# VatsalSy/gerris-fft-particles

Hardware: AMD Instinct MI355X
Metric: Mcell-steps/s (projection+advection), 3D 256^3 uniform (higher is better)
Workload: dtype f64; 1 GPU; 3-D periodic Taylor-Green, 256^3 per GPU, default projection/advection parameters (SURVEY 8d config C); relax_mode=exact, parallelism=1 box, rccl_world_size=0

## Files before the change

### gerris-fft-particles_amd/csrc/gfship_internal.hpp

```cpp
#pragma once

#include <hip/hip_runtime.h>
#include <cstdio>
#include <cstdarg>
#include <cstring>
#include <vector>
#include <deque>
#include <string>
#include <type_traits>
#include "gfship.h"
#include "switches.hpp"
#include "cell_update.hpp"

namespace gfship {

struct Layout {
  int n = 0;
  int px = 0;
  int xo = 1;
  int rows = 0;
  int dim = 3;
  long sy = 0;
  long sz = 0;
  size_t total = 0;
  __host__ __device__ inline long idx (int i, int j, int k) const {
    return xo + i + sy*j + sz*k;
  }
};

struct Field {
  bool used = false;
  int component = -1;
  double * lev[GFSHIP_MAXLEVEL + 1] = {};
  int bc[6] = {0, 0, 0, 0, 0, 0};
  double * bcval[6] = {};
// ... 69 lines not shown
  void * comm = nullptr;
  int overlap = 0;
  int lat_rank = -1, lat_n = 0, lat_b[3] = { 1, 1, 1 };
  gfship_gather_fn gather = nullptr; void * gather_ctx = nullptr;
  double * lat_res = nullptr, * lat_xch = nullptr;
  unsigned * lat_bar = nullptr;
  size_t lat_res_doubles = 0, lat_xch_doubles = 0;
  double * gfv_send[6] = {}, * gfv_recv[6] = {};
  double src[3] = { 0., 0., 0. };
  unsigned long long n_lattice_cycles = 0, n_fused_mpi = 0;
  unsigned long long kc[GFSHIP_KC_COUNT] = {};
  bool lattice_attr_set = false;
  void * mpi_plan[GFSHIP_MAXLEVEL + 1] = {};
  gfship_field dp_cache = -1;
  int skew_resident = -1;
  int patch_resident = 0;
  bool no_fused_godunov = false;
  bool no_fused_loop = false;
  bool force_hyperplane = false;
  bool unit_weights = false;
  bool weighted = false;
  unsigned long weights_stamp = 0;
  gfship_field wf[6] = {-1, -1, -1, -1, -1, -1};
  gfship::SkewPlan skew[GFSHIP_MAXLEVEL + 1];
  double diff_w[GFSHIP_MAXLEVEL + 1] = {};
  double * cfl_partial = nullptr;
  size_t cfl_nblocks = 0, cfl_used = 0;
  bool cfl_dirty = false;
  bool coarse_attr_set = false;
  gfship_field res_cache = -1;
  bool diff_ready = false;
  int diff_kind = 1;
  int patch_call = -1;
};

namespace gfship {

void set_error (const char * fmt, ...);
int  hip_fail (hipError_t e, const char * what, const char * file, int line);

inline int before_write (gfship_domain * dom)
{
  return dom->before_write ? dom->before_write (dom->before_write_ctx) : GFSHIP_OK;
}

#define GFSHIP_HIP(call) do { hipError_t e_ = (call); \
    if (e_ != hipSuccess) return gfship::hip_fail (e_, #call, __FILE__, __LINE__); } while (0)

inline hipError_t stream_wait_spin (hipStream_t st)
{
  hipError_t e;
  while ((e = hipStreamQuery (st)) == hipErrorNotReady)
    ;
  return e;
}

template <class F> inline void with_bools (F && f) { f (); }
template <class F, class... B> inline void with_bools (F && f, bool b0, B... rest)
{
  if (b0) with_bools ([&] (auto... r) { f (std::true_type {}, r...); }, rest...);
  else    with_bools ([&] (auto... r) { f (std::false_type {}, r...); }, rest...);
}

template <class F, class... B> inline void with_kind (F && f, int kind, B... bools)
{
  auto k = [&] (auto K) { with_bools ([&] (auto... r) { f (K, r...); }, bools...); };
// ... 52 lines not shown
			    int (* after_shell) (void *), void * ctx);
void mpi_order_free (gfship_domain * dom);
int launch_relax_loop_small (gfship_domain * dom, unsigned dimension, int level, double omega,
			     Field * dp, Field * ubc, const double * rhs, const double * dia,
			     unsigned nrelax, bool * done, const RelaxOp * op = nullptr);
int coarse_cycle_top (gfship_domain * dom, int minlevel);
int lattice_cycle_top (gfship_domain * dom, int minlevel, Field * dia);
int lattice_check_error (gfship_domain * dom);
int launch_lattice_cycle (gfship_domain * dom, unsigned dimension, double omega, int lmin, int ltop,
			  const unsigned * nrelax, Field * dp, Field * ubc, Field * res);
int launch_coarse_cycle (gfship_domain * dom, unsigned dimension, double omega, int lmin, int ltop,
			 const unsigned * nrelax, Field * dp, Field * ubc, Field * res, Field * dia);
int launch_relax_redblack (gfship_domain * dom, unsigned dimension, int level, double omega,
			   double * u, const double * rhs, const double * dia);
int launch_residual (gfship_domain * dom, int level, const double * u, const double * rhs,
		     const double * dia, double * res);
int launch_residual_weighted (gfship_domain * dom, int level, const double * u, const double * rhs,
			      const double * dia, double * res);
int launch_poisson_weights (gfship_domain * dom, double * const alpha[3]);
int launch_diffusion_weights (gfship_domain * dom, double * const D[3], double cdt);
int alloc_weights (gfship_domain * dom);
RelaxOp weighted_op (gfship_domain * dom, int level);
int launch_restrict (gfship_domain * dom, unsigned dimension, int level_coarse, double * v_coarse,
		     const double * v_fine);
int launch_prolongate (gfship_domain * dom, int level_coarse, const double * v_coarse,
		       double * v_fine);
int launch_correct (gfship_domain * dom, int level, double * u, const double * dp);
int launch_fill (gfship_domain * dom, int level, double * a, double value);
int launch_residual_norm (gfship_domain * dom, int level, const double * u, const double * rhs,
			  const double * dia, double * res, double scale, double weight,
			  double * out , bool dia_zero = false,
			  bool * store = nullptr );
int launch_norm_async (gfship_domain * dom, int level, const double * a, double scale, double weight);

int poisson_solve (gfship_domain * dom, gfship_multilevel_params * par, gfship_field lhs, gfship_field rhs,
		   gfship_field res, gfship_field dia, double dt, bool res_unread);
int launch_norm (gfship_domain * dom, int level, const double * a, double scale, double weight,
		 double out[5] );

int launch_face_interp_un (gfship_domain * dom, double * const u[3], double * const un[3]);
int launch_divergence (gfship_domain * dom, double * const un[3], double * div, double dt);
int launch_correct_un (gfship_domain * dom, const double * p, double * const un[3], double dt);
int launch_centered_gradient (gfship_domain * dom, const double * p, double * const g[3]);
int launch_correct_centered (gfship_domain * dom, double * const u[3], double * const g[3], double dt);
int launch_correct_centered_coarse (gfship_domain * dom, double * const u[3], double * const g[3],
				    double dt, double * const uc[3]);
int launch_coarse_init_from (gfship_domain * dom, Field * const * v, int nf, int top);
int launch_coarse_init_levels (gfship_domain * dom, Field * const * v, int nf, int top, int bottom);
int launch_advected_face_values (gfship_domain * dom, const double * v, double * const u[3],
				 double * const un[3], double dt, int use_centered, int gradient,
				 double * const fv[6], int cmask, double visc = 0., double gsrc = 0.,
				 const double * msrc = nullptr );
int launch_variable_mac_source (gfship_domain * dom, const double * v, double * const D[3],
				const double * alpha, double * out);
int launch_mac_source_fields (gfship_domain * dom, int c, const double * F, bool add_out, double * out);
int launch_centered_source_fields (gfship_domain * dom, double * v, const double * F, double gsrc, double dt);
int launch_face_bc (gfship_domain * dom, Field * v, double * const fv[6], int cmask);
int launch_predict_un (gfship_domain * dom, int cc, const double * uc, double * const fv[6],
		       double * unc);
int launch_flux_update (gfship_domain * dom, bool velocity, double * v, double * const un[3],
			double * const fv[6], const double * gm, const double * gc, double dt,
			double gsrc = 0.);
int launch_cfl (gfship_domain * dom, double * const u[3], double * const un[3],
		const double visc[3], double * cfl2,
		double * const msrc[3] = nullptr );
int launch_coarse_init (gfship_domain * dom, Field * const * v, int nf);
// ... 27 lines not shown
int  launch_relax_loop_skew (gfship_domain * dom, int level, Field * dp, Field * ubc,
			     const double * rhs, const double * dia, bool dia_zero,
			     unsigned nrelax, bool bc, double * correct_into = nullptr,
			     const double * prolong_from = nullptr, const RelaxOp * op = nullptr);
void skew_free (gfship_domain * dom);
bool skew_loop_supported (gfship_domain * dom, int level, unsigned nrelax, bool bc);
struct LoopGhosts;
int  skew_loop_run (gfship_domain * dom, int level, SkewPlan * S, double * u_nat, bool has_dia,
		    unsigned nrelax, float * ms = nullptr, const Field * ubc = nullptr,
		    const RelaxOp * op = nullptr, LoopGhosts * ghosts = nullptr);
int  skew_time_loop (gfship_domain * dom, int level, Field * u, const double * rhs,
		     const double * dia, bool dia_zero, unsigned nrelax, int reps,
		     double * ms_per_loop, int * fused, double * ms_inclusive = nullptr);
int  skew_check_error (gfship_domain * dom);
int  skew_arm_ahead (gfship_domain * dom, int level, unsigned nrelax);
int  patch_resident_per_cu (const gfship_domain * dom);
bool prolongation_fused (gfship_domain * dom, unsigned dimension, int level, unsigned nrelax);
bool prolongation_fusable (gfship_domain * dom, unsigned dimension, int level, unsigned nrelax);
bool line_prolongation_fused (gfship_domain * dom, unsigned dimension, int level, unsigned nrelax);
bool line_prolongation_fusable (gfship_domain * dom, unsigned dimension, int level, unsigned nrelax);
inline bool patch_level (const gfship_domain * dom, int level)
{
  const bool per_cell_weights = dom->patch_call < 0 ? dom->weighted : dom->patch_call == 0;
  return dom->sw.patch () && !per_cell_weights && dom->lay[level].n >= dom->sw.patch_min_n;
}
int  patch_pack (gfship_domain * dom, int level, SkewPlan * S, const double * u, const double * rhs,
		 const double * dia, const double * coarse = nullptr);
int  patch_unpack (gfship_domain * dom, int level, SkewPlan * S, double * u, double * add_into,
		   const LoopGhosts * ghosts = nullptr);
int  patch_restrict_pack (gfship_domain * dom, int level, SkewPlan * S, const double * res,
			  double * res_coarse, SkewPlan * Sc, unsigned dimension);
int  launch_restrict_pack (gfship_domain * dom, unsigned dimension, int level, Field * res,
			   bool coarse_fused);
void skew_dump_stats (gfship_domain * dom, int level);
int  skew_time_sweeps (gfship_domain * dom, int level, Field * u, const double * rhs,
		       const double * dia, bool dia_zero, int reps, double * ms_per_sweep);

}
```

### gerris-fft-particles_amd/csrc/poisson.hip

```cpp
#include "gfship_internal.hpp"
#include <cmath>
#include <cfloat>
#include <cstdlib>

using namespace gfship;

#define GFSHIP_CHECK_DIMENSION(dom, d) \
  GFSHIP_CHECK ((d) == (unsigned) (dom)->dim, GFSHIP_EUNSUPPORTED, \
		"dimension %u on a %d-D domain: only the dimension of the domain is implemented", (d), (dom)->dim)

namespace gfship {

static bool weighted_pipelinable (gfship_domain * dom, unsigned dimension, int level)
{
  return dom->relax_mode == GFSHIP_RELAX_EXACT && dimension == 3 && dom->dim == 3 &&
    skew_supported (dom, level) && !dom->force_hyperplane;
}

static bool weighted_pipelined (gfship_domain * dom, unsigned dimension, int level)
{
  return dom->sw.weighted_pipelined && weighted_pipelinable (dom, dimension, level);
}

static int relax_level (gfship_domain * dom, unsigned dimension, int level, double omega,
// ... 262 lines not shown

int gfship_norm_variable (gfship_domain * dom, gfship_field v, gfship_norm * out)
{
  Field * V = get_field (dom, v);
  if (!V || !out) return GFSHIP_EINVAL;
  const Layout & L = dom->lay[dom->depth];
  double size = 1./L.n;
  double vol = dom->dim == 3 ? size*size*size : size*size;
  double s[5];
  int r = launch_norm (dom, dom->depth, V->lev[dom->depth], 1., vol, s);
  if (r) return r;
  gfship_norm n;
  double wv = vol*(double) ncells (L);
  if (dom->has_external) {
    double sums[4] = { s[0], s[1], s[2], wv }, mx[1] = { s[3] };
    if ((r = call_reduce_norm (dom, sums, 4, mx))) return r;
    s[0] = sums[0]; s[1] = sums[1]; s[2] = sums[2]; wv = sums[3]; s[3] = mx[0];
  }
  n.bias = s[0]; n.first = s[1]; n.second = s[2]; n.infty = s[3];
  n.w = wv;
  if (n.w > 0.) {
    n.bias /= n.w;
    n.first /= n.w;
    n.second = sqrt (n.second/n.w);
  }
  else
    n.infty = 0.;
  *out = n;
  return GFSHIP_OK;
}

}

static int poisson_cycle (gfship_domain * dom, gfship_multilevel_params * p,
			  gfship_field u, gfship_field rhs, gfship_field dia, gfship_field res,
			  double dt, gfship_norm * norm, bool * store_res = nullptr)
{
  GFSHIP_CHECK (dom && p, GFSHIP_EINVAL, "null argument");
  GFSHIP_CHECK (p->dimension == 2 || p->dimension == 3, GFSHIP_EINVAL, "dimension must be 2 or 3");
  GFSHIP_CHECK_DIMENSION (dom, p->dimension);
  GFSHIP_CHECK (p->nrelax > 0 && p->erelax > 0, GFSHIP_EINVAL, "nrelax and erelax must be non zero");
  GFSHIP_CHECK (dom->unit_weights, GFSHIP_EINVAL, "call gfship_poisson_coefficients first");
  if (dom->dp_cache < 0)
    dom->dp_cache = gfship_field_alloc (dom, -1);
  gfship_field dpf = dom->dp_cache;
  if (dpf < 0) return dpf;
  Field * U = get_field (dom, u), * R = get_field (dom, rhs), * D = get_field (dom, dia),
    * S = get_field (dom, res), * DP = get_field (dom, dpf);
  int r = GFSHIP_OK;
  bool corrected = false;
  if (!U || !R || !D || !S) return GFSHIP_EINVAL;
  const int L = dom->depth;
  unsigned minlevel = p->minlevel;
  if (minlevel > (unsigned) L) minlevel = L;
  p->depth = L;

#define TRY(x) do { if ((r = (x)) != GFSHIP_OK) goto done; } while (0)
  for (int l = 0; l <= L; l++)
    S->zero[l] = U->zero[l] = false;
  {
    unsigned nrl[GFSHIP_MAXLEVEL + 1];
    {
      unsigned nr = p->nrelax;
      for (int l = L; l >= 0; l--) {
	nrl[l] = nr;
	if (l > (int) minlevel) nr *= p->erelax;
      }
    }
    for (int l = 0; l <= L; l++)
      DP->zero[l] = false;
    const int ctop = dom->weighted ? -1 : coarse_cycle_top (dom, (int) minlevel);
    const int ltop = ctop >= 0 ? -1 : lattice_cycle_top (dom, (int) minlevel, D);
    for (int l = L - 1; l >= (ctop >= 0 ? ctop + 1 : ltop >= 0 ? ltop : 0); l--) {
      if (dom->relax_mode == GFSHIP_RELAX_EXACT && p->dimension == 3 && !dom->weighted &&
	  !dom->force_hyperplane && skew_supported (dom, l + 1))
	TRY (skew_arm_ahead (dom, l + 1, nrl[l + 1]));
      const bool rp = !dom->skew[l + 1].rs_ready && prolongation_fused (dom, p->dimension, l + 1, nrl[l + 1]);
      if (rp) dom->kc[dom->sw.fused_restriction ? GFSHIP_KC_RESTRICTION_FUSED : GFSHIP_KC_RESTRICTION_DECLINED]++;
      if (dom->sw.fused_restriction && rp)
	TRY (launch_restrict_pack (dom, p->dimension, l + 1, S,
				   l > (int) minlevel && prolongation_fused (dom, p->dimension, l, nrl[l])));
      else
	TRY (launch_restrict (dom, p->dimension, l, S->lev[l], S->lev[l + 1]));
    }
    unsigned first = minlevel;
    if (ltop >= 0) {
      TRY (launch_lattice_cycle (dom, p->dimension, p->omega, (int) minlevel, ltop, nrl, DP, U, S));
      first = ltop + 1;
    }
    else if (ctop >= 0) {
      TRY (launch_coarse_cycle (dom, p->dimension, p->omega, (int) minlevel, ctop, nrl, DP, U, S, D));
      first = ctop + 1;
    }
    else {
      TRY (launch_fill (dom, minlevel, DP->lev[minlevel], 0.));
      TRY (relax_loop (dom, DP, U, p->dimension, minlevel, p->omega, S, D, nrl[minlevel]));
      first = minlevel + 1;
      dom->kc[GFSHIP_KC_COARSE_END_BY_LEVEL]++;
    }
    for (unsigned l = first; l <= p->depth; l++) {
      const bool fp = prolongation_fused (dom, p->dimension, (int) l, nrl[l]) ||
	line_prolongation_fused (dom, p->dimension, (int) l, nrl[l]);
      if (fp) dom->kc[GFSHIP_KC_PROLONGATION_FUSED]++;
      else if (prolongation_fusable (dom, p->dimension, (int) l, nrl[l]) ||
	       line_prolongation_fusable (dom, p->dimension, (int) l, nrl[l]))
	dom->kc[GFSHIP_KC_PROLONGATION_DECLINED]++;
      if (!fp)
	TRY (launch_prolongate (dom, l - 1, DP->lev[l - 1], DP->lev[l]));
      TRY (relax_loop (dom, DP, U, p->dimension, l, p->omega, S, D, nrl[l],
		       (int) l == L ? U->lev[L] : nullptr, &corrected, fp ? DP->lev[l - 1] : nullptr));
    }
  }
  if (!corrected)
    TRY (launch_correct (dom, L, U->lev[L], DP->lev[L]));
  if (!(corrected && all_sides_periodic (dom)))
    TRY (launch_bc (dom, U, U, L, 0));
  if (norm)
    TRY (residual_and_norm (dom, dt, U, R, D, S, norm, store_res));
  else if (dom->weighted)
    TRY (launch_residual_weighted (dom, L, U->lev[L], R->lev[L], D->lev[L], S->lev[L]));
  else
    TRY (launch_residual (dom, L, U->lev[L], R->lev[L], D->lev[L], S->lev[L]));
#undef TRY
 done:
  for (int l = 0; l <= L; l++)
    dom->skew[l].rs_ready = false;
  return r;
}

extern "C" {

int gfship_poisson_cycle (gfship_domain * dom, gfship_multilevel_params * p,
			  gfship_field u, gfship_field rhs, gfship_field dia, gfship_field res)
{
  GFSHIP_CHECK (dom != nullptr, GFSHIP_EINVAL, "null domain");
  int r = before_write (dom);
  if (r) return r;
  return poisson_cycle (dom, p, u, rhs, dia, res, 1., nullptr);
}

int gfship_poisson_solve (gfship_domain * dom, gfship_multilevel_params * par,
			  gfship_field lhs, gfship_field rhs, gfship_field res,
			  gfship_field dia, double dt)
{
  return poisson_solve (dom, par, lhs, rhs, res, dia, dt, false);
}

}

namespace gfship {

int poisson_solve (gfship_domain * dom, gfship_multilevel_params * par,
		   gfship_field lhs, gfship_field rhs, gfship_field res,
		   gfship_field dia, double dt, bool res_unread)
{
  GFSHIP_CHECK (dom && par, GFSHIP_EINVAL, "null argument");
  Field * U = get_field (dom, lhs), * R = get_field (dom, rhs), * D = get_field (dom, dia),
    * S = get_field (dom, res);
  if (!U || !R || !D || !S) return GFSHIP_EINVAL;
  GFSHIP_CHECK (par->dimension == 2 || par->dimension == 3, GFSHIP_EINVAL, "dimension must be 2 or 3");
  GFSHIP_CHECK_DIMENSION (dom, par->dimension);
  GFSHIP_CHECK (dom->unit_weights, GFSHIP_EINVAL, "call gfship_poisson_coefficients first");
  { int r = before_write (dom); if (r) return r; }
  int r;
  const int L = dom->depth;
  if ((r = coarse_flush (dom, U, L, true))) return r;
  unsigned minlevel = par->minlevel;
  par->depth = L;
  const unsigned predicted = res_unread ? par->niter : 0;
  bool res_stored = true;
  par->niter = 0;

  bool deferred = par->nitermin >= 1 && par->nitermax >= 1;
  if (deferred) {
    const Layout & Ly = dom->lay[L];
    double size = 1./Ly.n;
    S->zero[L] = false;
    if (dom->weighted) {
      if ((r = launch_residual_weighted (dom, L, U->lev[L], R->lev[L], D->lev[L], S->lev[L]))) return r;
      if ((r = launch_norm_async (dom, L, S->lev[L], 1.*size*size, 1.))) return r;
    }
    else if ((r = launch_residual_norm (dom, L, U->lev[L], R->lev[L], D->lev[L], S->lev[L], 1.*size*size,
					1., nullptr, D->zero[L])))
      return r;
  }
  else {
    if ((r = residual_and_norm (dom, dt, U, R, D, S, &par->residual))) return r;
    par->residual_before = par->residual;
  }

  double res_max_before = par->residual.infty;

  while (par->niter < par->nitermin ||
	 (par->residual.infty > par->tolerance && par->niter < par->nitermax)) {
    if (!res_stored) {
      if ((r = launch_residual (dom, L, U->lev[L], R->lev[L], D->lev[L], S->lev[L]))) break;
      res_stored = true;
    }
    bool store = !(predicted > 0 && par->niter + 1 == predicted);
    r = poisson_cycle (dom, par, lhs, rhs, dia, res, dt, &par->residual, &store);
    res_stored = store;
    if (r) {
      if (deferred) {
	deferred = false;
	double s0[5];
	if (hipStreamSynchronize (dom->stream) == hipSuccess) {
	  memcpy (s0, dom->h_pinned + 8, sizeof (s0));
	  if (norm_residual_finish (dom, dt, s0, &par->residual_before) == GFSHIP_OK)
	    par->residual = par->residual_before;
	}
	else
	  memset (&par->residual_before, 0, sizeof (par->residual_before)),
	    memset (&par->residual, 0, sizeof (par->residual));
      }
      break;
    }
    if (deferred) {
      deferred = false;
      double s0[5];
      memcpy (s0, dom->h_pinned + 8, sizeof (s0));
      if ((r = norm_residual_finish (dom, dt, s0, &par->residual_before))) break;
      res_max_before = par->residual_before.infty;
    }
    if (par->residual.infty == res_max_before)
      break;
    if (par->residual.infty > res_max_before/1.1 && par->minlevel < par->depth)
      par->minlevel++;
    res_max_before = par->residual.infty;
    par->niter++;
  }

  par->minlevel = minlevel;
  if (r == GFSHIP_OK)
// ... 68 lines not shown
```

### gerris-fft-particles_amd/csrc/poisson_kernels.hip

```cpp
#include "gfship_internal.hpp"
#include "cell_loop.hpp"
#include "relax_skew.hpp"
#include <algorithm>
#include <cstdlib>

namespace gfship {

template <int DIM, int OP>
__device__ __forceinline__ double relax_value (const double * __restrict__ u, long c, long sy, long sz,
					       double rhs, double dia, unsigned dimension,
					       double omega, double w, double h2, const W6 * wf = nullptr)
{
  return cell_update<DIM, OP> (kind_weights<OP> (w, ArrayW { wf, c }), ArrayU { u, c, sy, sz }, rhs, dia, u + c,
			       dimension, omega, h2);
}

__device__ __forceinline__ double relax_value_six (const double * __restrict__ u, long c, long sy, long sz,
						    double rhs)
{
  return cell_update_six (ArrayU { u, c, sy, sz }, rhs);
}

template <int DIM, int OP>
__global__ void __launch_bounds__(256)
// ... 1489 lines not shown
      s0 += weight*val;
      val = fabs (val);
      s3 = fmax (s3, val);
      s1 += weight*val;
      s2 += weight*val*val;
      s4 += raw;
    }
  }
  block_norm_sums (s0, s1, s2, s3, s4, partial, blockIdx.x);
}

__global__ void __launch_bounds__(256)
norm_final_kernel (const double * __restrict__ partial, int nblocks, double * __restrict__ out)
{
  double s0 = 0., s1 = 0., s2 = 0., s3 = 0., s4 = 0.;
  for (int q = threadIdx.x; q < nblocks; q += blockDim.x) {
    const double * p = partial + 5*(size_t) q;
    s0 += p[0]; s1 += p[1]; s2 += p[2]; s3 = fmax (s3, p[3]); s4 += p[4];
  }
  __shared__ double sh[5][4];
  s0 = wave_sum (s0); s1 = wave_sum (s1); s2 = wave_sum (s2); s3 = wave_max (s3); s4 = wave_sum (s4);
  int w = threadIdx.x >> 6, lane = threadIdx.x & 63;
  if (lane == 0) { sh[0][w] = s0; sh[1][w] = s1; sh[2][w] = s2; sh[3][w] = s3; sh[4][w] = s4; }
  __syncthreads ();
  if (threadIdx.x == 0) {
    double r0 = 0., r1 = 0., r2 = 0., r3 = 0., r4 = 0.;
    for (int q = 0; q < 4; q++) {
      r0 += sh[0][q]; r1 += sh[1][q]; r2 += sh[2][q]; r3 = fmax (r3, sh[3][q]); r4 += sh[4][q];
    }
    out[0] = r0; out[1] = r1; out[2] = r2; out[3] = r3; out[4] = r4;
  }
}

static bool power_of_two (double x)
{
  int e;
  return x > 0. && frexp (x, &e) == 0.5;
}
#define NORM_PARTIAL_LAUNCH() do {					\
    if (power_of_two (scale))						\
      hipLaunchKernelGGL (norm_partial_kernel<true>, dim3 (nblocks), dim3 (block), 0, dom->stream, \
			  L, a, scale, weight, partial);		\
    else								\
      hipLaunchKernelGGL (norm_partial_kernel<false>, dim3 (nblocks), dim3 (block), 0, dom->stream, \
			  L, a, scale, weight, partial);		\
  } while (0)

int launch_norm_async (gfship_domain * dom, int level, const double * a, double scale, double weight)
{
  const Layout & L = dom->lay[level];
  long nrows = L.dim == 3 ? (long) L.n*L.n : L.n;
  int block = L.n >= 256 ? 256 : L.n >= 128 ? 128 : 64;
  int nblocks = (int) (nrows > 1024 ? 1024 : nrows);
  double * partial = dom->d_scratch;
  double * result = dom->h_pinned + 8;
  NORM_PARTIAL_LAUNCH ();
  hipLaunchKernelGGL (norm_final_kernel, dim3 (1), dim3 (256), 0, dom->stream,
		      partial, nblocks, result);
  GFSHIP_HIP (hipGetLastError ());
  return GFSHIP_OK;
}

int launch_norm (gfship_domain * dom, int level, const double * a, double scale, double weight,
		 double out[5])
{
  const Layout & L = dom->lay[level];
  long nrows = L.dim == 3 ? (long) L.n*L.n : L.n;
  int block = L.n >= 256 ? 256 : L.n >= 128 ? 128 : 64;
  int nblocks = (int) (nrows > 1024 ? 1024 : nrows);
  double * partial = dom->d_scratch;
  double * result = dom->h_pinned;
// ... 96 lines not shown
  if (!NORM) return;
  __shared__ double sh[5][4];
  s0 = wave_sum (s0); s1 = wave_sum (s1); s2 = wave_sum (s2); s3 = wave_max (s3); s4 = wave_sum (s4);
  int w = threadIdx.x >> 6, lane = threadIdx.x & 63;
  if (lane == 0) { sh[0][w] = s0; sh[1][w] = s1; sh[2][w] = s2; sh[3][w] = s3; sh[4][w] = s4; }
  __syncthreads ();
  if (threadIdx.x == 0) {
    int nw = blockDim.x >> 6;
    double r0 = 0., r1 = 0., r2 = 0., r3 = 0., r4 = 0.;
    for (int q = 0; q < nw; q++) {
      r0 += sh[0][q]; r1 += sh[1][q]; r2 += sh[2][q]; r3 = fmax (r3, sh[3][q]); r4 += sh[4][q];
    }
    double * p = partial + 5*(size_t) blockIdx.x;
    p[0] = r0; p[1] = r1; p[2] = r2; p[3] = r3; p[4] = r4;
  }
}

int launch_residual_norm (gfship_domain * dom, int level, const double * u, const double * rhs,
			  const double * dia, double * res, double scale, double weight,
			  double * out, bool dia_zero, bool * store)
{
  const Layout & L = dom->lay[level];
  const bool no_store = store && !*store && power_of_two (scale) && dom->dim == 3 && L.n >= 64 &&
    dom->sw.residual_pairs;
  if (store) *store = !no_store;
  if (!power_of_two (scale)) {
    int r = launch_residual (dom, level, u, rhs, dia, res);
    if (r) return r;
    return out ? launch_norm (dom, level, res, scale, weight, out) :
      launch_norm_async (dom, level, res, scale, weight);
  }
  long nrows = L.dim == 3 ? (long) L.n*L.n : L.n;
  int block = L.n >= 256 ? 256 : L.n >= 128 ? 128 : 64;
  int rn_blocks = dom->sw.rn_blocks;
  if (rn_blocks < 64 || rn_blocks > 8192) rn_blocks = 4096;
  int nblocks = (int) (nrows > rn_blocks ? rn_blocks : nrows);
  double * partial = dom->d_scratch;
  double * result = out ? dom->h_pinned : dom->h_pinned + 8;
  const bool rn_pairs = dom->sw.residual_pairs;
  if (dom->dim == 3 && L.n >= 64) dom->kc[rn_pairs ? GFSHIP_KC_RESIDUAL_PAIRS : GFSHIP_KC_RESIDUAL_SCALAR]++;
  if (dom->dim == 3 && L.n >= 64 && rn_pairs) {
    const long nitems = (long) L.n*L.n*(L.n/2);
    long nb = (nitems + 255)/256;
    nblocks = (int) (nb > rn_blocks ? rn_blocks : nb);
    with_bools ([&] (auto ST) {
      hipLaunchKernelGGL ((residual_norm2_kernel<true, decltype (ST)::value>), dim3 (nblocks), dim3 (256), 0,
			  dom->stream, L, u, rhs, dia_zero ? nullptr : dia, res, 1./scale, weight, partial);
    }, !no_store);
  }
  else
    with_bools ([&] (auto D3) {
      hipLaunchKernelGGL (residual_norm_kernel<decltype (D3)::value ? 3 : 2>, dim3 (nblocks), dim3 (block), 0,
			  dom->stream, L, u, rhs, dia_zero ? nullptr : dia, res, 1./scale, weight, partial);
    }, dom->dim == 3);
  hipLaunchKernelGGL (norm_final_kernel, dim3 (1), dim3 (256), 0, dom->stream,
		      partial, nblocks, result);
  GFSHIP_HIP (hipGetLastError ());
  dom->kc[GFSHIP_KC_RN_BLOCKS_LIMIT] = rn_blocks;
  if ((unsigned long long) nblocks > dom->kc[GFSHIP_KC_RN_BLOCKS_MAX])
    dom->kc[GFSHIP_KC_RN_BLOCKS_MAX] = nblocks;
  if (out) {
    GFSHIP_HIP (stream_wait_spin (dom->stream));
    memcpy (out, dom->h_pinned, 5*sizeof (double));
  }
  return GFSHIP_OK;
}

struct MpiOrderPlan {
  int * cells = nullptr;
  std::vector<int> first;
  int shell_steps = 0;
};

template <int DIM, int OP>
__global__ void __launch_bounds__(256)
relax_listed_kernel (const int * __restrict__ cells, int count, long sy, long sz,
		     unsigned dimension, double omega, double w, double h2,
		     double * __restrict__ u, const double * __restrict__ rhs,
		     const double * __restrict__ dia)
{
  const int q = blockIdx.x*blockDim.x + threadIdx.x;
  if (q >= count) return;
  const long c = cells[q];
  u[c] = relax_value<DIM, OP> (u, c, sy, sz, rhs[c], dia[c], dimension, omega, w, h2);
}

static inline unsigned long long morton_key (int dim, int level, int I, int J, int K)
{
  unsigned long long m = 0;
  for (int b = level - 1; b >= 0; b--) {
    unsigned n = ((I >> b) & 1) | (((J >> b) & 1) << 1) | (dim == 3 ? ((K >> b) & 1) << 2 : 0);
    m = (m << (dim == 3 ? 3 : 2)) | n;
  }
  return m;
}

void mpi_order_free (gfship_domain * dom)
// ... 125 lines not shown
```

### gerris-fft-particles_amd/csrc/relax_patch_loop.hip

```cpp
#include "relax_skew.hpp"
#include <cstdlib>
#include <vector>

#ifndef PK_D
#define PK_D 9
#endif
#ifndef PK_DH
#define PK_DH 3
#endif
#ifndef PK_KO
#define PK_KO 0
#endif
#define PK_NTHREADS 192
#define PK_SKEW 14

namespace gfship {

typedef double d2 __attribute__((ext_vector_type(2)));

__device__ __forceinline__ void patch_arm_other_set (const SkewLoopArgs & A, int tile, int tid, int nt)
{
  if (A.arm_pairs == 0) return;
  typedef unsigned long long ull2 __attribute__((ext_vector_type(2)));
  const unsigned long long W = A.arm_cum[A.ntj*A.ntj];
  const unsigned long long lo = A.arm_pairs*A.arm_cum[tile]/W, hi = A.arm_pairs*A.arm_cum[tile + 1]/W;
  ull2 * const p = (ull2 *) A.arm;
  const ull2 ones = { ~0ull, ~0ull };
  for (unsigned long long i = lo + tid; i < hi; i += nt)
    __builtin_nontemporal_store (ones, p + i);
}

__device__ __forceinline__ unsigned patch_xcc_id ()
{
// ... 1008 lines not shown
    const int row = e / 32, col = e % 32;
    const int PA = col >> 2, p = col & 3;
    const int a = 2*PA + (p & 1), db = p >> 1;
    const int rho = r0 + row;
    const int I = rho - PA - PB;
    if (I >= 0 && I < n)
      A.dst[tbase + (long) rho*SK_NL + 128*(p >> 1) + 2*(PA + 8*PB) + (p & 1)] = buf[a + 16*db][I - I0];
  }
  for (int e = tid; e < 8*(PPR_ROWS/2); e += 256) {
    const int PA = e / (PPR_ROWS/2), mi = e % (PPR_ROWS/2);
    const int par = (PA + PB + r0) & 1;
    const int row = 2*mi + par;
    const int I = r0 + row - PA - PB;
    if (I >= 0 && I < n) {
      const int di = I - I0;
      double val = 0.;
#pragma unroll
      for (int id = 0; id < 8; id++)
	val += buf[2*PA + ((id >> 1) & 1) + 16*(id >> 2)][di + (id & 1)];
      const double v = A.dimension == 2 ? val : val/2.;
      const int m = I >> 1;
      const int pj = (n - SK_T*P - 2*PA) >> 1, pk = (n - SK_T*Q - 2*PB) >> 1;
      A.cnat[A.Lc.idx (m + 1, pj, pk)] = v;
      if (A.cskew) {
	const int ca = 8*(P & 1) + PA, cb = 8*(Q & 1) + PB;
	const long ctile = (P >> 1) + (long) A.cntj*(Q >> 1);
	A.cskew[ctile*(A.cRT + 2*SK_FP)*SK_NL + SK_FP*SK_NL +
		(long) (m + (ca >> 1) + (cb >> 1))*SK_NL + 128*(cb & 1) + 2*((ca >> 1) + 8*(cb >> 1)) + (ca & 1)] = v;
      }
    }
  }
}

__global__ void __launch_bounds__(256)
patch_unpack_kernel (PatchPackArgs A, LoopGhosts G)
{
  if ((int) blockIdx.z >= A.ntj*A.ntj) {
    loop_ghost_blocks (G, A.ntj*A.ntj);
    return;
  }
  __shared__ double buf[32][PPU_SPAN + 1];
  const int tid = threadIdx.x;
  const int tile = blockIdx.z, PB = blockIdx.y, r0 = blockIdx.x*PPU_ROWS;
  const int P = tile % A.ntj, Q = tile / A.ntj;
  const int n = A.L.n;
  const long tbase = (long) tile*(A.RT + 2*SK_FP)*SK_NL + SK_FP*SK_NL;
  const int I0 = r0 - 7 - PB;
  for (int e = tid; e < PPU_ROWS*32; e += 256) {
    const int row = e / 32, col = e % 32;
    const int PA = col >> 2, p = col & 3;
    const int a = 2*PA + (p & 1), db = p >> 1;
    const int rho = r0 + row;
    const int I = rho - PA - PB;
    if (I >= 0 && I < n)
      buf[a + 16*db][I - I0] = A.src[0][tbase + (long) rho*SK_NL + 128*(p >> 1) + 2*(PA + 8*PB) + (p & 1)];
  }
  __syncthreads ();
  for (int e = tid; e < 32*PPU_SPAN; e += 256) {
    const int line = e / PPU_SPAN, di = e % PPU_SPAN;
    const int a = line & 15, db = line >> 4;
    const int I = I0 + di;
    const int rho = I + (a >> 1) + PB;
    if (I >= 0 && I < n && rho >= r0 && rho < r0 + PPU_ROWS) {
      const int j = n - (SK_T*P + a), k = n - (SK_T*Q + 2*PB + db);
      const long c = A.L.idx (I + 1, j, k);
      if (A.add) {
// ... 44 lines not shown
    dim3 pgrid ((rows + PR_ROWS*PR_WAVES - 1)/(PR_ROWS*PR_WAVES), S->ntj*S->ntj);
    hipLaunchKernelGGL (patch_prolong_kernel, pgrid, dim3 (64*PR_WAVES), 0, dom->stream, Pr);
    GFSHIP_HIP (hipGetLastError ());
    if (A.narr == 1)
      return GFSHIP_OK;
    for (int q = 1; q < A.narr; q++) { A.src[q - 1] = A.src[q]; A.dst[q - 1] = A.dst[q]; }
    A.narr--;
    A.coarse = nullptr;
  }
  dim3 grid ((rows + PP_ROWS - 1)/PP_ROWS, 8, S->ntj*S->ntj);
  hipLaunchKernelGGL (patch_pack_kernel, grid, dim3 (256), 0, dom->stream, A);
  GFSHIP_HIP (hipGetLastError ());
  return GFSHIP_OK;
}

int patch_restrict_pack (gfship_domain * dom, int level, SkewPlan * S, const double * res,
			 double * res_coarse, SkewPlan * Sc, unsigned dimension)
{
  PatchRestrictArgs A;
  A.L = dom->lay[level]; A.Lc = dom->lay[level - 1];
  A.ntj = S->ntj; A.RT = S->RT;
  A.src = res; A.dst = S->rs;
  A.cnat = res_coarse;
  A.cskew = Sc ? Sc->rs : nullptr;
  A.cntj = Sc ? Sc->ntj : 0; A.cRT = Sc ? Sc->RT : 0;
  A.dimension = dimension;
  const int rows = A.L.n + PK_SKEW + 1;
  dim3 grid ((rows + PPR_ROWS - 1)/PPR_ROWS, 8, S->ntj*S->ntj);
  hipLaunchKernelGGL (patch_restrict_pack_kernel, grid, dim3 (256), 0, dom->stream, A);
  GFSHIP_HIP (hipGetLastError ());
  return GFSHIP_OK;
}

int patch_unpack (gfship_domain * dom, int level, SkewPlan * S, double * u, double * add_into,
		  const LoopGhosts * ghosts)
{
  PatchPackArgs A;
  A.coarse = nullptr; A.nat = nullptr; A.Lc = dom->lay[level];
  A.periodic = all_sides_periodic (dom);
  A.L = dom->lay[level]; A.ntj = S->ntj; A.RT = S->RT;
  A.narr = 1;
  A.src[0] = S->us; A.dst[0] = u; A.add = add_into;
  const int rows = A.L.n + PK_SKEW + 1;
  dim3 grid ((rows + PPU_ROWS - 1)/PPU_ROWS, 8, S->ntj*S->ntj);
  const LoopGhosts G = ghosts ? *ghosts : LoopGhosts ();
  grid.z += loop_ghost_planes (G, grid.x, grid.y);
  hipLaunchKernelGGL (patch_unpack_kernel, grid, dim3 (256), 0, dom->stream, A, G);
  GFSHIP_HIP (hipGetLastError ());
  return GFSHIP_OK;
}

int patch_loop_launch (gfship_domain * dom, const SkewLoopArgs & A, int ntiles, bool has_dia,
		       unsigned nrelax, float * ms, LoopGhosts * ghosts)
{
  if (ms) GFSHIP_HIP (hipEventRecord (dom->ev0, dom->stream));
  if (A.op == 1)
    hipLaunchKernelGGL ((relax_ring_loop_kernel<true, 1>), dim3 (ntiles), dim3 (RK_NTHREADS), 0, dom->stream, A);
  else if (dom->sw.patch_regs) {
    if (has_dia)
      hipLaunchKernelGGL (relax_patch_loop_kernel<true>, dim3 (ntiles), dim3 (PK_NTHREADS), 0, dom->stream, A);
    else
      hipLaunchKernelGGL (relax_patch_loop_kernel<false>, dim3 (ntiles), dim3 (PK_NTHREADS), 0, dom->stream, A);
  }
  else if (has_dia)
    hipLaunchKernelGGL ((relax_ring_loop_kernel<true, 0>), dim3 (ntiles), dim3 (RK_NTHREADS), 0, dom->stream, A);
  else
// ... 21 lines not shown
```

### gerris-fft-particles_amd/csrc/relax_skew.hip

```cpp
#include "relax_skew.hpp"
#include <cstdlib>

namespace gfship {

template <bool HAS_DIA>
__global__ void __launch_bounds__(SK_NL)
relax_skew_kernel (SkewArgs A)
{
  constexpr int XS = SK_T + 1;
  __shared__ double X[2][XS*XS];
  __shared__ double Y[2][XS*XS];
  __shared__ unsigned s_tile;

  const int tid = threadIdx.x;
  const int a = tid & (SK_T - 1), b = tid >> 4;
  const int n = A.L.n;
  const int ntj = A.ntj;
  const long tstride = (long) (A.RT + 2*SK_FP)*SK_NL;
  const long hstride = (long) SK_HROWS (n)*SK_T;

  if (tid == 0)
    s_tile = A.order[atomicAdd (A.ticket, 1u)];
  __syncthreads ();
  const int tile = s_tile;
// ... 520 lines not shown
			    const RelaxOp * op)
{
  SkewPlan * S;
  int r;
  if ((r = skew_plan (dom, level, &S))) return r;
  double * u = dp->lev[level];
  if ((r = skew_loop_trial (dom, level, S, nrelax, bc))) return r;
  if (op && op->kind >= 2) {
    if ((r = skew_pack_weights (dom, level, S, op))) return r;
    dia_zero = false;
  }
  const bool fusedp = prolong_from != nullptr && bc && (patch_level (dom, level) || all_sides_periodic (dom));
  const double * rhs_pack = S->rs_ready && patch_level (dom, level) ? nullptr : rhs;
  S->rs_ready = false;
  if (prolong_from && !fusedp)
    if ((r = launch_prolongate (dom, level - 1, prolong_from, u))) return r;
  if (fusedp && (r = skew_pack (dom, level, S, u, rhs_pack, dia_zero ? nullptr : dia, prolong_from))) return r;
  if (bc &&!(fusedp && prolong_images (dom, level)) && (r = launch_bc (dom, ubc, dp, level, 1))) return r;
  if (!fusedp && (r = skew_pack (dom, level, S, u, rhs_pack, dia_zero ? nullptr : dia))) return r;
  if (!dom->no_fused_loop && skew_loop_supported (dom, level, nrelax, bc)) {
    LoopGhosts G;
    const bool defer = all_sides_periodic (dom) && !op;
    if ((r = skew_loop_run (dom, level, S, u, !dia_zero, nrelax, nullptr, ubc, op, defer ? &G : nullptr))) return r;
    if (correct_into) G.active = false;
    return skew_unpack (dom, level, S, u, correct_into, &G);
  }
  for (unsigned q = 0; q < nrelax; q++) {
    if ((r = skew_sweep (dom, level, S, u, !dia_zero, op))) return r;
    if (bc && q + 1 < nrelax && (r = launch_bc (dom, ubc, dp, level, 1))) return r;
  }
  return skew_unpack (dom, level, S, u, correct_into);
}

int launch_restrict_pack (gfship_domain * dom, unsigned dimension, int level, Field * res, bool coarse_fused)
{
  SkewPlan * S, * Sc = nullptr;
  int r;
  if ((r = skew_plan (dom, level, &S))) return r;
  if ((r = skew_loop_trial (dom, level, S, 4, true))) return r;
  if (coarse_fused) {
    if ((r = skew_plan (dom, level - 1, &Sc))) return r;
    if ((r = skew_loop_trial (dom, level - 1, Sc, 4, true))) return r;
  }
  res->zero[level - 1] = false;
  if ((r = patch_restrict_pack (dom, level, S, res->lev[level], res->lev[level - 1], Sc, dimension))) return r;
  S->rs_ready = true;
  if (Sc) Sc->rs_ready = true;
  return GFSHIP_OK;
}

void skew_dump_stats (gfship_domain * dom, int level)
{
  SkewPlan & S = dom->skew[level];
  if (!S.stats) return;
  (void) hipStreamSynchronize (dom->stream);
  int nt = S.ntj*S.ntj;
  std::vector<u64> h (4*nt);
  (void) hipMemcpy (h.data (), S.stats, h.size ()*sizeof (u64), hipMemcpyDeviceToHost);
  u64 t0 = ~0ull;
  for (int q = 0; q < nt; q++) if (h[4*q] < t0) t0 = h[4*q];
  for (int Q = 0; Q < S.ntj; Q++)
    for (int P = 0; P < S.ntj; P++) {
      int q = P + S.ntj*Q;
      if (P == Q || P == 0 || Q == 0 || P == S.ntj - 1)
	fprintf (stderr, "tile (%2d,%2d) start %8.2f us  dur %8.2f us  spins %6llu slow %5llu\n", P, Q,
		 (h[4*q] - t0)/100., (h[4*q + 1] - h[4*q])/100., h[4*q + 2], h[4*q + 3]);
    }
}

int skew_time_sweeps (gfship_domain * dom, int level, Field * u, const double * rhs,
		      const double * dia, bool dia_zero, int reps, double * ms_per_sweep)
{
  SkewPlan * S;
  int r;
  if ((r = skew_plan (dom, level, &S))) return r;
  if ((r = skew_pack (dom, level, S, u->lev[level], rhs, dia_zero ? nullptr : dia))) return r;
  if ((r = skew_sweep (dom, level, S, u->lev[level], !dia_zero))) return r;
  float total = 0.f;
  for (int q = 0; q < reps; q++) {
    float ms = 0.f;
// ... 122 lines not shown
```

Baseline: 2872 Mcell-steps/s.

## Fuse finest-level residual, norm, restriction and skew pack into one kernel

When the residual is not read back, the finest-level residual computation is fused with the norm partial sums, the restriction to the coarse level, and the packing into the skewed tile layout. This happens in a single kernel, followed by a norm-final reduction. The following V-cycle then skips the separate restriction for that level via a restricted_level marker. The aim is to avoid writing the full fine residual array and reading it back for restriction, saving one full-grid memory pass per iteration. In exchange it adds complex index mapping, constant-coefficient assumptions (unit weights, zero diagonal), and cross-call state that must be reset correctly.

```diff
diff --git a/gerris-fft-particles_amd/csrc/gfship_internal.hpp b/gerris-fft-particles_amd/csrc/gfship_internal.hpp
--- a/gerris-fft-particles_amd/csrc/gfship_internal.hpp
+++ b/gerris-fft-particles_amd/csrc/gfship_internal.hpp
@@ -1,6 +1,7 @@
 #pragma once
 
 #include <hip/hip_runtime.h>
+#include <cmath>
 #include <cstdio>
 #include <cstdarg>
 #include <cstring>
@@ -136,6 +137,7 @@
   bool diff_ready = false;
   int diff_kind = 1;
   int patch_call = -1;
+  int restricted_level = -1;
 };
 
 namespace gfship {
@@ -254,6 +256,17 @@
 			  double * out , bool dia_zero = false,
 			  bool * store = nullptr );
 int launch_norm_async (gfship_domain * dom, int level, const double * a, double scale, double weight);
+int launch_residual_norm_final (gfship_domain * dom, int nblocks);
+inline int rn_blocks_limit (const gfship_domain * dom)
+{
+  const int rn_blocks = dom->sw.rn_blocks;
+  return rn_blocks < 64 || rn_blocks > 8192 ? 4096 : rn_blocks;
+}
+inline bool power_of_two (double x)
+{
+  int e;
+  return x > 0. && frexp (x, &e) == 0.5;
+}
 
 int poisson_solve (gfship_domain * dom, gfship_multilevel_params * par, gfship_field lhs, gfship_field rhs,
 		   gfship_field res, gfship_field dia, double dt, bool res_unread);
@@ -347,6 +360,11 @@
 			  double * res_coarse, SkewPlan * Sc, unsigned dimension);
 int  launch_restrict_pack (gfship_domain * dom, unsigned dimension, int level, Field * res,
 			   bool coarse_fused);
+int  patch_residual_restrict_pack (gfship_domain * dom, int level, SkewPlan * S, const double * u,
+				   const double * rhs, double * res_coarse, SkewPlan * Sc, unsigned dimension,
+				   double scale, double weight, int * nblocks);
+int  launch_residual_restrict_pack (gfship_domain * dom, unsigned dimension, int level, const double * u,
+				    const double * rhs, Field * res, bool coarse_fused, double scale, double weight);
 void skew_dump_stats (gfship_domain * dom, int level);
 int  skew_time_sweeps (gfship_domain * dom, int level, Field * u, const double * rhs,
 		       const double * dia, bool dia_zero, int reps, double * ms_per_sweep);
diff --git a/gerris-fft-particles_amd/csrc/poisson.hip b/gerris-fft-particles_amd/csrc/poisson.hip
--- a/gerris-fft-particles_amd/csrc/poisson.hip
+++ b/gerris-fft-particles_amd/csrc/poisson.hip
@@ -318,6 +318,47 @@
 
 }
 
+struct CyclePlan {
+  unsigned minlevel;
+  unsigned nrl[GFSHIP_MAXLEVEL + 1];
+  int ctop, ltop;
+  int lowest;
+};
+
+static CyclePlan cycle_plan (gfship_domain * dom, const gfship_multilevel_params * p, Field * D)
+{
+  CyclePlan C;
+  const int L = dom->depth;
+  C.minlevel = p->minlevel;
+  if (C.minlevel > (unsigned) L) C.minlevel = L;
+  unsigned nr = p->nrelax;
+  for (int l = L; l >= 0; l--) {
+    C.nrl[l] = nr;
+    if (l > (int) C.minlevel) nr *= p->erelax;
+  }
+  C.ctop = dom->weighted ? -1 : coarse_cycle_top (dom, (int) C.minlevel);
+  C.ltop = C.ctop >= 0 ? -1 : lattice_cycle_top (dom, (int) C.minlevel, D);
+  C.lowest = C.ctop >= 0 ? C.ctop + 1 : C.ltop >= 0 ? C.ltop : 0;
+  return C;
+}
+
+static bool cycle_restrict_packs (gfship_domain * dom, unsigned dimension, const CyclePlan & C, int fine)
+{
+  return fine - 1 >= C.lowest && prolongation_fused (dom, dimension, fine, C.nrl[fine]);
+}
+
+static bool cycle_restrict_packs_coarse (gfship_domain * dom, unsigned dimension, const CyclePlan & C, int fine)
+{
+  return fine - 1 > (int) C.minlevel && prolongation_fused (dom, dimension, fine - 1, C.nrl[fine - 1]);
+}
+
+static void cycle_state_reset (gfship_domain * dom)
+{
+  for (int l = 0; l <= dom->depth; l++)
+    dom->skew[l].rs_ready = false;
+  dom->restricted_level = -1;
+}
+
 static int poisson_cycle (gfship_domain * dom, gfship_multilevel_params * p,
 			  gfship_field u, gfship_field rhs, gfship_field dia, gfship_field res,
 			  double dt, gfship_norm * norm, bool * store_res = nullptr)
@@ -337,35 +378,29 @@
   bool corrected = false;
   if (!U || !R || !D || !S) return GFSHIP_EINVAL;
   const int L = dom->depth;
-  unsigned minlevel = p->minlevel;
-  if (minlevel > (unsigned) L) minlevel = L;
   p->depth = L;
 
 #define TRY(x) do { if ((r = (x)) != GFSHIP_OK) goto done; } while (0)
   for (int l = 0; l <= L; l++)
     S->zero[l] = U->zero[l] = false;
   {
-    unsigned nrl[GFSHIP_MAXLEVEL + 1];
-    {
-      unsigned nr = p->nrelax;
-      for (int l = L; l >= 0; l--) {
-	nrl[l] = nr;
-	if (l > (int) minlevel) nr *= p->erelax;
-      }
-    }
+    const CyclePlan C = cycle_plan (dom, p, D);
+    const unsigned minlevel = C.minlevel;
+    const unsigned * const nrl = C.nrl;
+    const int ctop = C.ctop, ltop = C.ltop;
     for (int l = 0; l <= L; l++)
       DP->zero[l] = false;
-    const int ctop = dom->weighted ? -1 : coarse_cycle_top (dom, (int) minlevel);
-    const int ltop = ctop >= 0 ? -1 : lattice_cycle_top (dom, (int) minlevel, D);
-    for (int l = L - 1; l >= (ctop >= 0 ? ctop + 1 : ltop >= 0 ? ltop : 0); l--) {
+    for (int l = L - 1; l >= C.lowest; l--) {
       if (dom->relax_mode == GFSHIP_RELAX_EXACT && p->dimension == 3 && !dom->weighted &&
 	  !dom->force_hyperplane && skew_supported (dom, l + 1))
 	TRY (skew_arm_ahead (dom, l + 1, nrl[l + 1]));
-      const bool rp = !dom->skew[l + 1].rs_ready && prolongation_fused (dom, p->dimension, l + 1, nrl[l + 1]);
+      if (dom->restricted_level == l + 1)
+	continue;
+      const bool rp = !dom->skew[l + 1].rs_ready && cycle_restrict_packs (dom, p->dimension, C, l + 1);
       if (rp) dom->kc[dom->sw.fused_restriction ? GFSHIP_KC_RESTRICTION_FUSED : GFSHIP_KC_RESTRICTION_DECLINED]++;
       if (dom->sw.fused_restriction && rp)
 	TRY (launch_restrict_pack (dom, p->dimension, l + 1, S,
-				   l > (int) minlevel && prolongation_fused (dom, p->dimension, l, nrl[l])));
+				   cycle_restrict_packs_coarse (dom, p->dimension, C, l + 1)));
       else
 	TRY (launch_restrict (dom, p->dimension, l, S->lev[l], S->lev[l + 1]));
     }
@@ -409,8 +444,7 @@
     TRY (launch_residual (dom, L, U->lev[L], R->lev[L], D->lev[L], S->lev[L]));
 #undef TRY
  done:
-  for (int l = 0; l <= L; l++)
-    dom->skew[l].rs_ready = false;
+  cycle_state_reset (dom);
   return r;
 }
 
@@ -466,6 +500,20 @@
       if ((r = launch_residual_weighted (dom, L, U->lev[L], R->lev[L], D->lev[L], S->lev[L]))) return r;
       if ((r = launch_norm_async (dom, L, S->lev[L], 1.*size*size, 1.))) return r;
     }
+    else if (res_unread && par->dimension == 3 && dom->sw.residual_pairs && dom->sw.fused_restriction &&
+	     power_of_two (1.*size*size) && Ly.n >= 64 && D->zero[L] && par->nrelax > 0 && par->erelax > 0 &&
+	     par->minlevel < (unsigned) L) {
+      const CyclePlan C = cycle_plan (dom, par, D);
+      if (cycle_restrict_packs (dom, par->dimension, C, L)) {
+	dom->kc[GFSHIP_KC_RESTRICTION_FUSED]++;
+	r = launch_residual_restrict_pack (dom, par->dimension, L, U->lev[L], R->lev[L], S,
+					   cycle_restrict_packs_coarse (dom, par->dimension, C, L), 1.*size*size, 1.);
+      }
+      else
+	r = launch_residual_norm (dom, L, U->lev[L], R->lev[L], D->lev[L], S->lev[L], 1.*size*size, 1., nullptr,
+				  D->zero[L]);
+      if (r) { cycle_state_reset (dom); return r; }
+    }
     else if ((r = launch_residual_norm (dom, L, U->lev[L], R->lev[L], D->lev[L], S->lev[L], 1.*size*size,
 					1., nullptr, D->zero[L])))
       return r;
@@ -485,6 +533,7 @@
     }
     bool store = !(predicted > 0 && par->niter + 1 == predicted);
     r = poisson_cycle (dom, par, lhs, rhs, dia, res, dt, &par->residual, &store);
+    cycle_state_reset (dom);
     res_stored = store;
     if (r) {
       if (deferred) {
diff --git a/gerris-fft-particles_amd/csrc/poisson_kernels.hip b/gerris-fft-particles_amd/csrc/poisson_kernels.hip
--- a/gerris-fft-particles_amd/csrc/poisson_kernels.hip
+++ b/gerris-fft-particles_amd/csrc/poisson_kernels.hip
@@ -1545,11 +1545,6 @@
   }
 }
 
-static bool power_of_two (double x)
-{
-  int e;
-  return x > 0. && frexp (x, &e) == 0.5;
-}
 #define NORM_PARTIAL_LAUNCH() do {					\
     if (power_of_two (scale))						\
       hipLaunchKernelGGL (norm_partial_kernel<true>, dim3 (nblocks), dim3 (block), 0, dom->stream, \
@@ -1712,8 +1707,7 @@
   }
   long nrows = L.dim == 3 ? (long) L.n*L.n : L.n;
   int block = L.n >= 256 ? 256 : L.n >= 128 ? 128 : 64;
-  int rn_blocks = dom->sw.rn_blocks;
-  if (rn_blocks < 64 || rn_blocks > 8192) rn_blocks = 4096;
+  const int rn_blocks = rn_blocks_limit (dom);
   int nblocks = (int) (nrows > rn_blocks ? rn_blocks : nrows);
   double * partial = dom->d_scratch;
   double * result = out ? dom->h_pinned : dom->h_pinned + 8;
@@ -1743,6 +1737,17 @@
     GFSHIP_HIP (stream_wait_spin (dom->stream));
     memcpy (out, dom->h_pinned, 5*sizeof (double));
   }
+  return GFSHIP_OK;
+}
+
+int launch_residual_norm_final (gfship_domain * dom, int nblocks)
+{
+  hipLaunchKernelGGL (norm_final_kernel, dim3 (1), dim3 (256), 0, dom->stream,
+		      dom->d_scratch, nblocks, dom->h_pinned + 8);
+  GFSHIP_HIP (hipGetLastError ());
+  dom->kc[GFSHIP_KC_RN_BLOCKS_LIMIT] = rn_blocks_limit (dom);
+  if ((unsigned long long) nblocks > dom->kc[GFSHIP_KC_RN_BLOCKS_MAX])
+    dom->kc[GFSHIP_KC_RN_BLOCKS_MAX] = nblocks;
   return GFSHIP_OK;
 }
 
diff --git a/gerris-fft-particles_amd/csrc/relax_patch_loop.hip b/gerris-fft-particles_amd/csrc/relax_patch_loop.hip
--- a/gerris-fft-particles_amd/csrc/relax_patch_loop.hip
+++ b/gerris-fft-particles_amd/csrc/relax_patch_loop.hip
@@ -1,4 +1,6 @@
 #include "relax_skew.hpp"
+#include "cell_loop.hpp"
+#include "residual_pack_map.hpp"
 #include <cstdlib>
 #include <vector>
 
@@ -1073,6 +1075,121 @@
   }
 }
 
+struct ResidualRestrictArgs {
+  PatchRestrictArgs R;
+  const double * u, * rhs;
+  double inv, weight;
+  double * partial;
+  int nrb;
+  int ntasks;
+};
+
+#define RRP_PAIRS (PPR_ROWS/2 + 1)
+#define RRP_W (PPR_SPAN + 1)
+
+template <bool NORM>
+__global__ void __launch_bounds__(256)
+residual_restrict_pack_kernel (ResidualRestrictArgs B)
+{
+  __shared__ __attribute__((aligned(16))) double buf[32][RRP_W];
+  const PatchRestrictArgs & A = B.R;
+  const int tid = threadIdx.x;
+  const int n = A.L.n, ntiles = A.ntj*A.ntj;
+  double s0 = 0., s1 = 0., s2 = 0., s3 = 0., s4 = 0.;
+  for (int t = blockIdx.x; t < B.ntasks; t += gridDim.x) {
+    const ResidualRestrictTask T = residual_restrict_task (t, B.nrb);
+    if (T.tile < ntiles) {
+      const int tile = T.tile, PB = T.PB, r0 = T.rb*PPR_ROWS;
+      const int P = tile % A.ntj, Q = tile / A.ntj;
+      const long tbase = (long) tile*(A.RT + 2*SK_FP)*SK_NL + SK_FP*SK_NL;
+      const int I0 = residual_restrict_origin (r0, PB);
+      for (int e = tid; e < 32*RRP_PAIRS; e += 256) {
+	const ResidualRestrictPair pr = residual_restrict_pair<PPR_ROWS> (e, r0, PB);
+	if (residual_restrict_pair_needed<PPR_ROWS> (pr, n)) {
+	  const int I = pr.I;
+	  const int j = n - (SK_T*P + pr.a), k = n - (SK_T*Q + 2*PB + pr.db);
+	  const double * __restrict__ u = B.u;
+	  const long c = A.L.idx (I + 1, j, k);
+	  const d2 uc = *(const d2 *) (u + c);
+	  const double ul = u[c - 1], ur = u[c + 2];
+	  const d2 ut = *(const d2 *) (u + c + A.L.sy), ub = *(const d2 *) (u + c - A.L.sy);
+	  const d2 uf = *(const d2 *) (u + c + A.L.sz), uk = *(const d2 *) (u + c - A.L.sz);
+	  const d2 rh = *(const d2 *) (B.rhs + c);
+	  d2 out;
+	  {
+	    double sa = 0., sb = 0.;
+	    sa += 1.; sb += 1.*uc.y;
+	    sa += 1.; sb += 1.*ul;
+	    sa += 1.; sb += 1.*ut.x;
+	    sa += 1.; sb += 1.*ub.x;
+	    sa += 1.; sb += 1.*uf.x;
+	    sa += 1.; sb += 1.*uk.x;
+	    out.x = rh.x - (sb - uc.x*sa);
+	  }
+	  {
+	    double sa = 0., sb = 0.;
+	    sa += 1.; sb += 1.*ur;
+	    sa += 1.; sb += 1.*uc.x;
+	    sa += 1.; sb += 1.*ut.y;
+	    sa += 1.; sb += 1.*ub.y;
+	    sa += 1.; sb += 1.*uf.y;
+	    sa += 1.; sb += 1.*uk.y;
+	    out.y = rh.y - (sb - uc.y*sa);
+	  }
+	  *(d2 *) &buf[pr.line][I - I0] = out;
+	  if (NORM)
+#pragma unroll
+	    for (int q = 0; q < 2; q++)
+	      if (residual_restrict_owns<PPR_ROWS> (pr, q)) {
+		const double raw = q ? out.y : out.x;
+		double val = raw*B.inv;
+		s0 += B.weight*val;
+		val = fabs (val);
+		s3 = fmax (s3, val);
+		s1 += B.weight*val;
+		s2 += B.weight*val*val;
+		s4 += raw;
+	      }
+	}
+      }
+      __syncthreads ();
+      for (int e = tid; e < PPR_ROWS*32; e += 256) {
+	const int row = e / 32, col = e % 32;
+	const int PA = col >> 2, p = col & 3;
+	const int a = 2*PA + (p & 1), db = p >> 1;
+	const int rho = r0 + row;
+	const int I = rho - PA - PB;
+	if (I >= 0 && I < n)
+	  A.dst[tbase + (long) rho*SK_NL + 128*(p >> 1) + 2*(PA + 8*PB) + (p & 1)] = buf[a + 16*db][I - I0];
+      }
+      for (int e = tid; e < 8*(PPR_ROWS/2); e += 256) {
+	const ResidualRestrictCoarse cc = residual_restrict_coarse<PPR_ROWS> (e, r0, PB);
+	const int PA = cc.PA, I = cc.I;
+	if (I >= 0 && I < n) {
+	  const int di = I - I0;
+	  double val = 0.;
+#pragma unroll
+	  for (int id = 0; id < 8; id++)
+	    val += buf[2*PA + ((id >> 1) & 1) + 16*(id >> 2)][di + (id & 1)];
+	  const double v = A.dimension == 2 ? val : val/2.;
+	  const int m = I >> 1;
+	  const int pj = (n - SK_T*P - 2*PA) >> 1, pk = (n - SK_T*Q - 2*PB) >> 1;
+	  A.cnat[A.Lc.idx (m + 1, pj, pk)] = v;
+	  if (A.cskew) {
+	    const int ca = 8*(P & 1) + PA, cb = 8*(Q & 1) + PB;
+	    const long ctile = (P >> 1) + (long) A.cntj*(Q >> 1);
+	    A.cskew[ctile*(A.cRT + 2*SK_FP)*SK_NL + SK_FP*SK_NL +
+		    (long) (m + (ca >> 1) + (cb >> 1))*SK_NL + 128*(cb & 1) + 2*((ca >> 1) + 8*(cb >> 1)) + (ca & 1)] = v;
+	  }
+	}
+      }
+    }
+    __syncthreads ();
+  }
+  if (NORM)
+    block_norm_sums (s0, s1, s2, s3, s4, B.partial, blockIdx.x);
+}
+
 __global__ void __launch_bounds__(256)
 patch_unpack_kernel (PatchPackArgs A, LoopGhosts G)
 {
@@ -1183,6 +1300,32 @@
   return GFSHIP_OK;
 }
 
+int patch_residual_restrict_pack (gfship_domain * dom, int level, SkewPlan * S, const double * u,
+				  const double * rhs, double * res_coarse, SkewPlan * Sc, unsigned dimension,
+				  double scale, double weight, int * nblocks)
+{
+  ResidualRestrictArgs B;
+  PatchRestrictArgs & A = B.R;
+  A.L = dom->lay[level]; A.Lc = dom->lay[level - 1];
+  A.ntj = S->ntj; A.RT = S->RT;
+  A.src = nullptr; A.dst = S->rs;
+  A.cnat = res_coarse;
+  A.cskew = Sc ? Sc->rs : nullptr;
+  A.cntj = Sc ? Sc->ntj : 0; A.cRT = Sc ? Sc->RT : 0;
+  A.dimension = dimension;
+  B.u = u; B.rhs = rhs;
+  B.inv = 1./scale; B.weight = weight;
+  B.partial = dom->d_scratch;
+  const int rows = A.L.n + PK_SKEW + 1;
+  B.nrb = (rows + PPR_ROWS - 1)/PPR_ROWS;
+  B.ntasks = residual_restrict_ntasks (B.nrb, S->ntj*S->ntj);
+  const int limit = rn_blocks_limit (dom);
+  *nblocks = B.ntasks > limit ? limit : B.ntasks;
+  hipLaunchKernelGGL (residual_restrict_pack_kernel<true>, dim3 (*nblocks), dim3 (256), 0, dom->stream, B);
+  GFSHIP_HIP (hipGetLastError ());
+  return GFSHIP_OK;
+}
+
 int patch_unpack (gfship_domain * dom, int level, SkewPlan * S, double * u, double * add_into,
 		  const LoopGhosts * ghosts)
 {
diff --git a/gerris-fft-particles_amd/csrc/relax_skew.hip b/gerris-fft-particles_amd/csrc/relax_skew.hip
--- a/gerris-fft-particles_amd/csrc/relax_skew.hip
+++ b/gerris-fft-particles_amd/csrc/relax_skew.hip
@@ -576,20 +576,44 @@
   return skew_unpack (dom, level, S, u, correct_into);
 }
 
+static int restrict_pack_plans (gfship_domain * dom, int level, bool coarse_fused, SkewPlan ** S, SkewPlan ** Sc)
+{
+  int r;
+  *Sc = nullptr;
+  if ((r = skew_plan (dom, level, S))) return r;
+  if ((r = skew_loop_trial (dom, level, *S, 4, true))) return r;
+  if (coarse_fused) {
+    if ((r = skew_plan (dom, level - 1, Sc))) return r;
+    if ((r = skew_loop_trial (dom, level - 1, *Sc, 4, true))) return r;
+  }
+  return GFSHIP_OK;
+}
+
 int launch_restrict_pack (gfship_domain * dom, unsigned dimension, int level, Field * res, bool coarse_fused)
 {
-  SkewPlan * S, * Sc = nullptr;
+  SkewPlan * S, * Sc;
   int r;
-  if ((r = skew_plan (dom, level, &S))) return r;
-  if ((r = skew_loop_trial (dom, level, S, 4, true))) return r;
-  if (coarse_fused) {
-    if ((r = skew_plan (dom, level - 1, &Sc))) return r;
-    if ((r = skew_loop_trial (dom, level - 1, Sc, 4, true))) return r;
-  }
+  if ((r = restrict_pack_plans (dom, level, coarse_fused, &S, &Sc))) return r;
   res->zero[level - 1] = false;
   if ((r = patch_restrict_pack (dom, level, S, res->lev[level], res->lev[level - 1], Sc, dimension))) return r;
   S->rs_ready = true;
   if (Sc) Sc->rs_ready = true;
+  return GFSHIP_OK;
+}
+
+int launch_residual_restrict_pack (gfship_domain * dom, unsigned dimension, int level, const double * u,
+				   const double * rhs, Field * res, bool coarse_fused, double scale, double weight)
+{
+  SkewPlan * S, * Sc;
+  int r, nblocks = 0;
+  if ((r = restrict_pack_plans (dom, level, coarse_fused, &S, &Sc))) return r;
+  res->zero[level - 1] = false;
+  if ((r = patch_residual_restrict_pack (dom, level, S, u, rhs, res->lev[level - 1], Sc, dimension,
+					 scale, weight, &nblocks))) return r;
+  if ((r = launch_residual_norm_final (dom, nblocks))) return r;
+  S->rs_ready = true;
+  if (Sc) Sc->rs_ready = true;
+  dom->restricted_level = level;
   return GFSHIP_OK;
 }
 
diff --git a/gerris-fft-particles_amd/csrc/residual_pack_map.hpp b/gerris-fft-particles_amd/csrc/residual_pack_map.hpp
--- /dev/null
+++ b/gerris-fft-particles_amd/csrc/residual_pack_map.hpp
@@ -0,0 +1,66 @@
+#pragma once
+
+namespace gfship {
+
+struct ResidualRestrictTask { int tile, PB, rb; };
+
+__host__ __device__ inline int residual_restrict_ntasks (int nrb, int ntiles)
+{
+  return 64*((nrb*ntiles + 7)/8);
+}
+
+__host__ __device__ inline ResidualRestrictTask residual_restrict_task (int t, int nrb)
+{
+  ResidualRestrictTask T;
+  const int idx = (t & 7) + 8*(t >> 6);
+  T.PB = (t >> 3) & 7;
+  T.rb = idx % nrb;
+  T.tile = idx / nrb;
+  return T;
+}
+
+struct ResidualRestrictPair { int line, a, db, lo, I; };
+
+template <int ROWS>
+__host__ __device__ inline ResidualRestrictPair residual_restrict_pair (int e, int r0, int PB)
+{
+  ResidualRestrictPair p;
+  const int pi = e % (ROWS/2 + 1);
+  p.line = e / (ROWS/2 + 1);
+  p.a = p.line & 15; p.db = p.line >> 4;
+  p.lo = r0 - (p.a >> 1) - PB;
+  p.I = (p.lo & ~1) + 2*pi;
+  return p;
+}
+
+template <int ROWS>
+__host__ __device__ inline bool residual_restrict_pair_needed (const ResidualRestrictPair & p, int n)
+{
+  return p.I >= 0 && p.I < n && p.I < p.lo + ROWS;
+}
+
+template <int ROWS>
+__host__ __device__ inline bool residual_restrict_owns (const ResidualRestrictPair & p, int q)
+{
+  return p.I + q >= p.lo && p.I + q < p.lo + ROWS;
+}
+
+__host__ __device__ inline int residual_restrict_origin (int r0, int PB)
+{
+  return (r0 - 7 - PB) & ~1;
+}
+
+struct ResidualRestrictCoarse { int PA, I; };
+
+template <int ROWS>
+__host__ __device__ inline ResidualRestrictCoarse residual_restrict_coarse (int e, int r0, int PB)
+{
+  ResidualRestrictCoarse c;
+  c.PA = e / (ROWS/2);
+  const int mi = e % (ROWS/2);
+  const int par = (c.PA + PB + r0) & 1;
+  c.I = r0 + 2*mi + par - c.PA - PB;
+  return c;
+}
+
+}
```

Result: faster. 2923 Mcell-steps/s, median of 6 (+1.8%).
